# AdriaJ/pyxu

Hardware: AMD Instinct MI355X
Metric: solver iterations/s (PGD, TV-regularised deblur) (higher is better)
Workload: dtype f32; 1 GPU; PGD 2048x2048 Gaussian(sigma=2) deblur + lam*env_mu(L21 o Grad) TV, PositiveOrthant; images_per_gpu=1, stop_crit=MaxIter | RelError, fused_m_step=True, pgd_launch=x, x_prev, H^T y -> x_new (tile kernel), parallelism=independent images x1 (one per rank)

## Files before the change

include/pyxu_amd.h:

```cpp
#ifndef PYXU_AMD_H
#define PYXU_AMD_H

#include <stddef.h>
#include <stdint.h>

#ifdef __cplusplus
extern "C" {
#endif

#define PXA_F32 0
#define PXA_F64 1

#define PXA_OK 0
#define PXA_ERR_ARG (-1)
#define PXA_ERR_DTYPE (-2)
#define PXA_ERR_UNSUPPORTED (-3)

#define PXA_MAX_DIM 4
#define PXA_MAX_TAPS 64

#define PXA_MODE_CONSTANT 0
#define PXA_MODE_WRAP 1
#define PXA_MODE_REFLECT 2
#define PXA_MODE_SYMMETRIC 3
// ... 233 lines not shown
int pxa_pgd_tv2d_plan_step(void* plan, double a, double tau, double prox_w, const void* x, const void* x_prev,
                           const void* hty, void* x_new, double* partials, const void* x_ref, double* rel_values,
                           uint32_t* rel_flags, uint32_t seq, void* stream);
int pxa_pgd_tv2d_plan_step_fold(void* plan, double a, double tau, double prox_w, const void* x, const void* x_prev,
                                const void* hty, void* x_new, double* partials, const void* x_ref, double* rel_values,
                                uint32_t* rel_flags, uint32_t seq, void* stream);
int pxa_pgd_tv2d_plan_step_wfold(void* plan, double a, double tau, double prox_w, const void* x, const void* x_prev,
                                 const void* hty, void* x_new, double* partials, double* rel_values, uint32_t* rel_flags,
                                 uint32_t seq, void* stream);
int pxa_pgd_tv2d_plan_step_wpub(void* plan, double a, double tau, double prox_w, const void* x, const void* x_prev,
                                const void* hty, void* x_new, double* partials, const double* prev_partials,
                                double* rel_values, uint32_t* rel_flags, uint32_t seq, void* stream);
int pxa_pgd_tv2d_plan_free(void* plan);
int pxa_pgd_tv2d_last_kernel(void);
int pxa_pgd_tile_trace(uint64_t* host_out, int n);
int pxa_pgd_tv2d_step(int dtype, int64_t stack, int64_t y_images, int64_t n0, int64_t n1, int nt0, const int32_t* off0,
                      const double* coef0, int nt1, const int32_t* off1, const double* coef1, double h0, double h1,
                      double lam, double mu, double a, double tau, int prox, double prox_w, const void* x,
                      const void* x_prev, const void* hty, void* x_new, double* partials, const void* x_ref,
                      void* stream);


int pxa_fft(int dtype, int ndim, const int64_t* shape, int naxes, const int* axes, int64_t stack, int inverse,
            const void* in, void* out, void* stream);
size_t pxa_fft_workspace_bytes(int dtype, int ndim, const int64_t* shape, int naxes, const int* axes, int64_t stack);
int pxa_fft_ex(int dtype, int ndim, const int64_t* shape, int naxes, const int* axes, int64_t stack, int inverse,
               const void* in, void* out, void* work, void* stream);
int pxa_complex_mul(int dtype, int64_t n, int64_t nb, const void* a, const void* b, int conj_b, void* out,
                    void* stream);
int pxa_real_to_complex(int dtype, int64_t n, const void* x, void* z, void* stream);
// ... 35 lines not shown

int pxa_pds_slab_primal(int dtype, int algo, const int64_t* geom, const int32_t* ntaps, const int32_t* offs,
                        const double* coefs, const double* diff, const double* scal, int prox, int h_kind,
                        const void* x, const void* u, const void* z, const void* hty, void* x_out, void* u_out,
                        void* work_q, void* work_w, const int64_t* ghost, const void* src_lo, const void* src_hi,
                        const void* z_lo, const void* z_hi, int nseg, void* stream);
int pxa_pds_slab_dual(int dtype, int relax, const int64_t* geom, const double* diff, double sigma, double lam,
                      double rho, int h_kind, const void* w, const void* w_hi, int64_t w_hi_depth, const void* z,
                      void* z_out, void* stream);

int pxa_pds_step_la(int dtype, int algo, const int64_t* geom, const int32_t* ntaps, const int32_t* offs,
                    const double* coefs, const double* diff, const double* scal, int prox, int h_kind, int primed,
                    void* x, const void* u, const void* z, const void* hty, void* x_out, void* u_out, void* z_out,
                    void* work_q, void* work_kt, void* work_w, int nseg, void* stream);

#ifdef __cplusplus
}
#endif

#endif
```

pyxu_amd/_lib.py:

```python
import ctypes as ct
import os
import threading

__all__ = ["lib", "check", "BackendUnavailable", "LIB_PATH", "EXPORTS"]

LIB_PATH = os.environ.get("PXA_LIB_PATH") or os.path.join(os.path.dirname(os.path.abspath(__file__)), "libpyxu_amd.so")

i32, i64, f64, vp, sz = ct.c_int, ct.c_int64, ct.c_double, ct.c_void_p, ct.c_size_t
P_i64 = ct.POINTER(ct.c_int64)
P_i32 = ct.POINTER(ct.c_int32)
P_int = ct.POINTER(ct.c_int)
P_f64 = ct.POINTER(ct.c_double)

EXPORTS = {
    "pxa_version": (ct.c_char_p, []),
    "pxa_error_string": (ct.c_char_p, [i32]),
    "pxa_abi_version": (i32, []),
    "pxa_tuning": (i32, [i32, i32]),
    "pxa_axpby": (i32, [i32, i64, f64, vp, f64, vp, vp, vp]),
    "pxa_axpby_bcast": (i32, [i32, i64, f64, vp, f64, vp, i64, vp, vp]),
    "pxa_axpy_rows": (i32, [i32, i64, i64, vp, f64, vp, vp, vp, vp]),
    "pxa_row_ratio": (i32, [i32, i64, vp, vp, vp, vp]),
    "pxa_lincomb3": (i32, [i32, i64, f64, vp, f64, vp, f64, vp, vp, vp]),
    "pxa_extrapolate": (i32, [i32, i64, f64, vp, vp, vp, vp]),
# ... 56 lines not shown
    "pxa_dense_normal_pdot": (i32, [i32, i64, i64, vp, vp, f64, f64, vp, vp, vp, vp]),
    "pxa_dense_normal_pdot_pfold": (i32, [i32, i64, i64, vp, vp, vp, vp, vp, vp, vp, vp, vp, ct.c_uint32, f64, f64, vp, vp,
                                          vp, vp]),
    "pxa_copy2d": (i32, [i32, i64, i64, vp, i64, i64, vp, i64, i32, vp]),
    "pxa_unary": (i32, [i32, i32, i64, vp, vp, vp]),
    "pxa_binary": (i32, [i32, i32, i64, vp, f64, vp, f64, vp, vp]),
    "pxa_where": (i32, [i32, i64, vp, vp, f64, vp, f64, vp, vp]),
    "pxa_cast": (i32, [i32, i32, i64, vp, vp, vp]),
    "pxa_isnan": (i32, [i32, i64, vp, vp, vp]),
    "pxa_bool_reduce": (i32, [i64, i32, vp, vp, vp]),
    "pxa_set_diag": (i32, [i32, i64, i64, i64, f64, vp, vp]),
    "pxa_transpose": (i32, [i32, i64, i64, vp, vp, vp]),
    "pxa_dir_contract": (i32, [i32, i64, i64, i64, i64, i64, vp, i64, vp, vp, i32, vp]),
    "pxa_pgd_tv2d_partials_count": (i32, [i64, i64, i64]),
    "pxa_pgd_tv2d_last_kernel": (i32, []),
    "pxa_pgd_tile_trace": (i32, [vp, i32]),
    "pxa_pgd_tv2d_plan": (i32, [i32, i64, i64, i64, i64, i32, P_i32, P_f64, i32, P_i32, P_f64, f64, f64, f64, f64, i32,
                                ct.POINTER(vp)]),
    "pxa_pgd_tv2d_plan_step": (i32, [vp, f64, f64, f64, vp, vp, vp, vp, vp, vp, vp, vp, ct.c_uint32, vp]),
    "pxa_pgd_tv2d_plan_step_fold": (i32, [vp, f64, f64, f64, vp, vp, vp, vp, vp, vp, vp, vp, ct.c_uint32, vp]),
    "pxa_pgd_tv2d_plan_step_wfold": (i32, [vp, f64, f64, f64, vp, vp, vp, vp, vp, vp, vp, ct.c_uint32, vp]),
    "pxa_pgd_tv2d_plan_step_wpub": (i32, [vp, f64, f64, f64, vp, vp, vp, vp, vp, vp, vp, vp, ct.c_uint32, vp]),
    "pxa_pgd_tv2d_plan_free": (i32, [vp]),
    "pxa_pgd_tv2d_step": (
        i32,
        [i32, i64, i64, i64, i64, i32, P_i32, P_f64, i32, P_i32, P_f64, f64, f64, f64, f64, f64, f64, i32, f64,
         vp, vp, vp, vp, vp, vp, vp],
    ),
    "pxa_fft": (i32, [i32, i32, P_i64, i32, P_int, i64, i32, vp, vp, vp]),
    "pxa_fft_workspace_bytes": (sz, [i32, i32, P_i64, i32, P_int, i64]),
    "pxa_fft_ex": (i32, [i32, i32, P_i64, i32, P_int, i64, i32, vp, vp, vp, vp]),
# ... 106 lines not shown
```

pyxu_amd/csrc/pgd_tv2d.hip:

```cpp
#include "tile2d.hpp"
#include <type_traits>

#ifndef PXA_PGD_PRIO
#define PXA_PGD_PRIO 1
#endif
#ifndef PXA_PGD_PRIO_EPI
#define PXA_PGD_PRIO_EPI 0
#endif
#ifndef PXA_PGD_PRIO_FIN
#define PXA_PGD_PRIO_FIN 0
#endif

#ifndef PXA_PROBES
#define PXA_PROBES 0
#endif

namespace pxa {
namespace {

using namespace tile2d;
constexpr bool kProbes = PXA_PROBES != 0;


template <typename T>
// ... 12 lines not shown
  int diag;
  const T* xref;
  double* fold_vals;
  unsigned* fold_flags;
  unsigned* counter;
  unsigned fold_seq;
  int64_t fold_rows, fold_per_row;
  int win_part;
  const double* pub_src;
  double* pub_vals;
  unsigned* pub_flags;
  unsigned pub_seq;
};


constexpr int kTraceWords = 4 * 4 * 8;
__device__ unsigned long long g_tile_trace[kTraceWords];

template <typename T>
__device__ inline T tv_weight(T n2, T lam, T mu, T inv_mu) {
  const T n = sqrt(n2);
  return lam / (n > mu ? n : mu);
}
template <>
__device__ inline float tv_weight<float>(float n2, float lam, float mu, float inv_mu) {
  const float r = __builtin_amdgcn_rsqf(n2);
  return lam * __builtin_fminf(r, inv_mu);
}

template <typename T, int R>
struct Window {
  using L = Layout<T, R>;
// ... 59 lines not shown
    for (int i = 0; i < L::N0; ++i)
      if (cnt[i] != 1) return false;
    return true;
  }
  static_assert(covers_once(), "the window order is a bijection onto the AR x NGA window vectors");

  T xv[K0][L::V], pv[K0][L::V];
};

__device__ inline void wave_lane(int lt, int& wv, int& ln) {
  wv = __builtin_amdgcn_readfirstlane(lt >> 6);
  __builtin_assume(wv >= 0 && wv < kThreads / 64);
  ln = lt & 63;
}

constexpr int kMaxInteriorN1 = 1 << 22;
template <typename T>
__device__ inline T* lane_ptr(T* img, int row0, int col0, int n1, int ru, unsigned voff) {
  T* base = img + ((int64_t)row0 * n1 + col0) + ru * n1;
  using C = std::conditional_t<std::is_const_v<T>, const char, char>;
  return reinterpret_cast<T*>(reinterpret_cast<C*>(base) + (size_t)voff);
}

template <typename T, int R, bool EDGE>
__device__ inline void win_issue(const PgdParams<T>& p, int ty0, int tx0, const T* __restrict__ xs,
                                 const T* __restrict__ xps, Window<T, R>& w, int lt) {
  using L = Layout<T, R>;
  using W = Window<T, R>;
  constexpr int V = L::V;
  constexpr int CA = L::CA;
  const int n0 = p.n0, n1 = p.n1;
  int wv, ln;
  wave_lane(lt, wv, ln);
#pragma unroll
  for (int k = 0; k < W::K0; ++k) {
    int rl, gl, ru, gu;
    if (W::item(k, wv, ln, rl, gl, ru, gu)) {
      if (!EDGE) {
        const unsigned voff = (unsigned)(rl * n1 + V * gl) * (unsigned)sizeof(T);
        ld_vec<T, V>(lane_ptr<const T>(xs, ty0 - 2 * R, tx0 - CA + V * gu, n1, ru, voff), w.xv[k]);
        if (kProbes && (p.diag & 256)) {
#pragma unroll
          for (int v = 0; v < V; ++v) w.pv[k][v] = w.xv[k][v];
        } else {
          ld_vec<T, V>(lane_ptr<const T>(xps, ty0 - 2 * R, tx0 - CA + V * gu, n1, ru, voff), w.pv[k]);
        }
        continue;
      }
      const int gr = ty0 - 2 * R + rl + ru, gc = tx0 - CA + V * (gl + gu);
      if (gr >= 0 && gr < n0 && p.vec_ok && gc >= 0 && gc + V <= n1) {
        ld_vec<T, V>(xs + (int64_t)gr * n1 + gc, w.xv[k]);
        ld_vec<T, V>(xps + (int64_t)gr * n1 + gc, w.pv[k]);
      } else {
// ... 21 lines not shown
    if (W::item(k, wv, ln, rl, gl, ru, gu)) {
      T out[V];
#pragma unroll
      for (int v = 0; v < V; ++v) out[v] = fma(w.xv[k][v] - w.pv[k][v], p.a, w.xv[k][v]);
      st_vec<T, V>(A + (rl * L::AP + V * gl) + (ru * L::AP + V * gu), out);
    }
  }
}

template <typename T, int R>
__host__ __device__ constexpr int pt_pitch() {
  if constexpr (sizeof(T) == 4) return BlockB<T, R>::PTP;
  else return Layout<T, R>::PTP;
}

template <typename T, int R, bool EDGE, int D = 0>
__device__ inline void pass_a(const PgdParams<T>& p, const T* A, T* PT, const T* KT, int ty0, int tid = threadIdx.x) {
  using L = Layout<T, R>;
  constexpr int V = L::V;
  constexpr int KA = cdiv(L::NPA, kThreads);
  const bool edge_rows = EDGE && (ty0 < R || ty0 + TY > p.n0 - R);
#pragma unroll
  for (int k = 0; k < KA; ++k) {
    const int it = tid + k * kThreads;
    if (it < L::NPA) {
      const int a = it % L::NA, b = it / L::NA;
      T acc[V][V];
      sweep<T, R, V, L::AP, D>(A + (V * a) * L::AP + V * b, p.g0, acc);
      if (edge_rows) ghost_fix<T, R, V, L::AP>(ty0 + V * a, p.n0, ty0 - 2 * R, A + V * b, p.k0, KT, acc);
#pragma unroll
      for (int v = 0; v < V; ++v) {
        T colv[V];
#pragma unroll
        for (int u = 0; u < V; ++u) colv[u] = acc[u][v];
        st_vec<T, V>(PT + (V * b + v) * pt_pitch<T, R>() + V * a, colv);
      }
    }
  }
}

__device__ inline void st_pair(float* p, float a, float b) { *reinterpret_cast<float2*>(p) = make_float2(a, b); }

constexpr int kTvxP0 = 40;
template <typename T, int R>
constexpr int kTvxFloats = 9 * kTvxP0 + 9 * BlockB<T, R>::WR;

template <typename T, int R, bool EDGE>
__device__ inline void tv_block(const PgdParams<T>& p, T* A, int ty0, int tx0, int wv, int ln, T (&yc)[2][4],
                                T (&tv)[2][4]) {
  using L = Layout<T, R>;
  using B = BlockB<T, R>;
  constexpr int CA = L::CA, AP = L::AP;
  constexpr bool kExchange = (2 * R - 1) * AP >= 2 * kTvxFloats<T, R>;
  const int n0 = p.n0, n1 = p.n1;
  int rpl, cil, wr0, wc0;
  B::item(wv, ln, rpl, cil, wr0, wc0);
  const int r0 = wr0 + 2 * rpl, c0 = wc0 + 4 * cil;
  const T* own = A + (r0 + 2 * R) * AP + CA + c0;
  auto qat = [&](T yc_, T ydn, T yrt, int gr, int gc, T& q0, T& q1) {
    const T v0 = fma(p.g0a, yc_, p.g0b * ydn);
    const T v1 = fma(p.g1a, yc_, p.g1b * yrt);
    T w = tv_weight<T>(fma(v0, v0, v1 * v1), p.lam, p.mu, p.inv_mu);
    if (EDGE && !(gr >= 0 && gr < n0 && gc >= 0 && gc < n1)) w = T(0);
    q0 = v0 * w;
    q1 = v1 * w;
  };
  if constexpr (kExchange) {
    T y[3][5];
#pragma unroll
    for (int r = 0; r < 3; ++r) {
      T m[4];
      ld_vec<T, 4>(own + r * AP, m);
#pragma unroll
      for (int w = 0; w < 4; ++w) y[r][w] = m[w];
    }
#pragma unroll
    for (int r = 0; r < 2; ++r) {
      T hi[2];
// ... 6 lines not shown
      for (int w = 0; w < 4; ++w) yc[u][w] = y[u][w];
    if (!p.tv) return;
    T q0[2][4], q1[2][4];
#pragma unroll
    for (int u = 0; u < 2; ++u)
#pragma unroll
      for (int w = 0; w < 4; ++w)
        qat(y[u][w], y[u + 1][w], y[u][w + 1], ty0 + r0 + u, tx0 + c0 + w, q0[u][w], q1[u][w]);
    T* E0 = (wv < 2 ? A : A + (TY + 2 * R + 1) * AP) + (wv & 1) * kTvxFloats<T, R>;
    T* E1 = E0 + 9 * kTvxP0;
    if (ln < 48) {
      T hq0, hq1;
      if (ln < 32) {
        const int tc = wc0 + ln;
        const T* h = A + (wr0 - 1 + 2 * R) * AP + CA + tc;
        qat(h[0], h[AP], h[1], ty0 + wr0 - 1, tx0 + tc, hq0, hq1);
        E0[ln] = hq0;
      } else {
        const int j = ln - 32, tc = wc0 - 1;
        const T* h = A + (wr0 + j + 2 * R) * AP + CA + tc;
        qat(h[0], h[AP], h[1], ty0 + wr0 + j, tx0 + tc, hq0, hq1);
        E1[j] = hq1;
      }
    }
    st_vec<T, 4>(E0 + (rpl + 1) * kTvxP0 + 4 * cil, q0[1]);
    st_pair(E1 + (cil + 1) * B::WR + 2 * rpl, q1[0][3], q1[1][3]);
    __builtin_amdgcn_wave_barrier();
    asm volatile("" ::: "memory");
    T up[4], left[2];
    ld_vec<T, 4>(E0 + rpl * kTvxP0 + 4 * cil, up);
    ld_pair<T>(E1 + cil * B::WR + 2 * rpl, left);
#pragma unroll
    for (int u = 0; u < 2; ++u)
#pragma unroll
      for (int w = 0; w < 4; ++w) {
        const T qa = u == 0 ? up[w] : q0[0][w];
// ... 2 lines not shown
        const T t1 = fma(p.g1b, ql, p.g1a * q1[u][w]);
        tv[u][w] = t0 + t1;
      }
  } else {
    auto yrow = [&](int r, T(&y)[6]) {
      const T* arow = own + (r - 1) * AP;
      T m[4];
      ld_vec<T, 4>(arow, m);
      y[0] = arow[-1];
#pragma unroll
      for (int w = 0; w < 4; ++w) y[w + 1] = m[w];
      y[5] = arow[4];
    };
    auto qrow = [&](int r, const T(&yr)[6], const T(&yn)[6], T(&q0)[5], T(&q1)[5]) {
#pragma unroll
      for (int c = 0; c < 5; ++c) qat(yr[c], yn[c], yr[c + 1], ty0 + r0 - 1 + r, tx0 + c0 - 1 + c, q0[c], q1[c]);
    };
    T yr[6], yn[6];
    yrow(0, yr);
    yrow(1, yn);
    T qp0[5], qp1[5];
    if (p.tv) qrow(0, yr, yn, qp0, qp1);
#pragma unroll
    for (int u = 0; u < 2; ++u) {
#pragma unroll
      for (int c = 0; c < 6; ++c) yr[c] = yn[c];
      yrow(u + 2, yn);
#pragma unroll
      for (int w = 0; w < 4; ++w) yc[u][w] = yr[w + 1];
      if (p.tv) {
        T qc0[5], qc1[5];
// ... 188 lines not shown
#pragma unroll
  for (int off = 32; off > 0; off >>= 1) {
    part_d += __shfl_down(part_d, off, 64);
    part_x += __shfl_down(part_x, off, 64);
  }
  if ((threadIdx.x & 63) == 0) {
    __hip_atomic_store(partials + 2 * slot, part_d, __ATOMIC_RELAXED, __HIP_MEMORY_SCOPE_AGENT);
    __hip_atomic_store(partials + 2 * slot + 1, part_x, __ATOMIC_RELAXED, __HIP_MEMORY_SCOPE_AGENT);
  }
}

template <int R>
constexpr bool kRowsLiveB = R >= 4;
constexpr int kRingB = 4;

template <typename T, int R, bool EDGE, typename Mark>
__device__ inline void pass_b_blocks(const PgdParams<T>& p, T* A, const T* PT, const T* KT, const T* GH, int ty0, int tx0,
                                     const T* __restrict__ bs, const T* __restrict__ xrs, T* __restrict__ xns,
                                     bool want_part, double& part_d, double& part_x, int tid, Mark&& tmark) {
  using L = Layout<T, R>;
  using B = BlockB<T, R>;
  constexpr int CA = L::CA, PTP = B::PTP;
  const int n0 = p.n0, n1 = p.n1;
  const bool edge_cols = EDGE && (tx0 < R || tx0 + TX > n1 - R);
  int wv, ln;
  wave_lane(tid, wv, ln);
  int rpl, cil, wr0, wc0;
  B::item(wv, ln, rpl, cil, wr0, wc0);
  const int r0 = wr0 + 2 * rpl, c0 = wc0 + 4 * cil;
  auto voff = [&](int q) { return (unsigned)((2 * rpl + q) * n1 + 4 * cil) * (unsigned)sizeof(T); };
  auto load_rows = [&](const T* __restrict__ src, T(&v)[2][4]) {
#pragma unroll
    for (int q = 0; q < 2; ++q) {
      const int gr = ty0 + r0 + q, gc = tx0 + c0;
      if (!EDGE) {
        ld_vec<T, 4>(lane_ptr<const T>(src, ty0, tx0 + wc0, n1, wr0, voff(q)), v[q]);
      } else if (vec_inside(p, gr, gc)) {
// ... 14 lines not shown
    } else {
      load_rows(bs, bv);
    }
  };
  T yc[2][4], tv[2][4], acc[4][2];
  if (kProbes && (p.diag & 64)) {
#pragma unroll
    for (int q = 0; q < 2; ++q)
#pragma unroll
      for (int w = 0; w < 4; ++w) yc[q][w] = tv[q][w] = acc[w][q] = A[tid + q * 64 + w];
    load_epilogue();
    tmark(5);
  } else {
    const T* src = PT + (CA - 2 * R + c0) * PTP + r0;
    if constexpr (kRowsLiveB<R>) {
      tv_block<T, R, EDGE>(p, A, ty0, tx0, wv, ln, yc, tv);
      tmark(5);
      load_epilogue();
      sweep_w<T, R, 4, 2, PTP>(src, p.g1, acc);
    } else {
      T g1[4 * R + 1];
#pragma unroll
      for (int k = 0; k <= 4 * R; ++k) {
        g1[k] = p.g1[k];
        asm volatile("" : "+s"(g1[k]));
      }
      RowSweep<T, R, 4, 2, PTP, kRingB> sw;
      tv_block<T, R, EDGE>(p, A, ty0, tx0, wv, ln, yc, tv);
      tmark(5);
      load_epilogue();
      sw.start(src);
      sw.run(src, g1, acc);
    }
    if (edge_cols) ghost_fix_pre_w<T, R, 4, 2, TY>(tx0 + c0, n1, r0, GH, KT + kKT, acc);
  }
  if (want_part) load_rows(xrs, xv);
  tmark(6);
#pragma unroll
  for (int q = 0; q < 2; ++q) {
    T g[4];
#pragma unroll
    for (int w = 0; w < 4; ++w) g[w] = p.tv ? acc[w][q] + tv[q][w] : acc[w][q];
    if (kProbes && (p.diag & 1024)) {
      if (g[0] + yc[q][0] + bv[q][0] == T(-12345)) xns[0] = T(0);
      continue;
    }
    T* vdst = EDGE ? nullptr : lane_ptr<T>(xns, ty0, tx0 + wc0, n1, wr0, voff(q));
    finish_vec<T, EDGE>(p, ty0 + r0 + q, tx0 + c0, g, bv[q], yc[q], xv[q], xns, vdst, want_part, part_d, part_x);
  }
// ... 80 lines not shown
      ld_vec<T, V>(A + (r + 2 * R) * L::AP + L::CA + V * cq, y);
      if (kProbes && (p.diag & 1024)) {
        if (g[0] + y[0] + hb.v[s][0] == T(-12345)) xns[0] = T(0);
        continue;
      }
      T* vdst = EDGE ? nullptr : lane_ptr<T>(xns, ty0, tx0, n1, 0, stage_voff<T, R>(r0, cq, n1, s));
      finish_vec<T, EDGE>(p, ty0 + r, tx0 + V * cq, g, hb.v[s], y, hb.x[s], xns, vdst, want_part, part_d, part_x);
    }
  }
}

#ifndef PXA_PGD_SWEEP_DEPTH
#define PXA_PGD_SWEEP_DEPTH 0
#endif

template <typename T, int R, bool EDGE, int D>
__device__ inline void pgd_tile_body(const PgdParams<T>& p, unsigned char* smem, unsigned tile, int ty0, int tx0,
                                     const T* __restrict__ bs, T* __restrict__ xns, double* __restrict__ partials,
                                     const T* __restrict__ xrs, const int tid) {
  using L = Layout<T, R>;
  T* A = reinterpret_cast<T*>(smem);
  T* PT = A + L::AR * L::AP;
  T* KT = PT + L::AC * L::PTP;
  T* GH = reinterpret_cast<T*>(smem + kGhOff<T, R>);
  const int n1 = p.n1;
  const bool edge_cols = EDGE && (tx0 < R || tx0 + TX > n1 - R);
  double part_d = 0.0, part_x = 0.0;
  const bool want_part = partials != nullptr;
  const bool tracing = kProbes && (p.diag & 32) != 0;
  unsigned long long* ts = reinterpret_cast<unsigned long long*>(smem + kGhOff<T, R> + kGhBytes<T, R>);
  auto tmark = [&](int pt) {
    if (tracing && (tid & 63) == 0) ts[(tid >> 6) * 8 + pt] = clock64();
  };
  tmark(2);
  const bool skip_passes = kProbes && (p.diag & 64) != 0;
  if (!skip_passes) pass_a<T, R, EDGE, D>(p, A, PT, KT, ty0, tid);
  tmark(3);
  __syncthreads();
  if (edge_cols) {
    ghost_cols_coop<T, R, pt_pitch<T, R>()>(p.k1, PT, GH, tx0, n1, tid);
    __syncthreads();
  }
  tmark(4);
  if constexpr (sizeof(T) == 4) {
    pass_b_blocks<T, R, EDGE>(p, A, PT, KT, GH, ty0, tx0, bs, xrs, xns, want_part, part_d, part_x, tid, tmark);
  } else {
    pass_b_staged<T, R, EDGE, D>(p, A, PT, KT, GH, ty0, tx0, bs, xrs, xns, want_part, part_d, part_x, tid, tmark);
  }
  tmark(7);
  if (want_part) wave_partials(part_d, part_x, partials, tile * kPartWaves + (tid >> 6));
  const unsigned nb = gridDim.x, bid = blockIdx.x;
  if (tracing && (bid == 0 || bid == 9 || bid == nb / 2 + 8 || bid == nb - 1)) {
    __syncthreads();
    const int slot = bid == 0 ? 0 : bid == 9 ? 1 : bid == nb / 2 + 8 ? 2 : 3;
    if (tid < 32) g_tile_trace[slot * 32 + tid] = ts[tid];
  }
}


template <typename T, int R>
__device__ inline void win_partials(const Window<T, R>& w, double* __restrict__ partials, unsigned tile, const int tid) {
  using L = Layout<T, R>;
  double part_d = 0.0, part_x = 0.0;
#pragma unroll
  for (int k = 0; k < Window<T, R>::KI; ++k) {
#pragma unroll
    for (int v = 0; v < L::V; ++v) {
      const double dd = (double)w.xv[k][v] - (double)w.pv[k][v];
      part_d = fma(dd, dd, part_d);
      part_x = fma((double)w.pv[k][v], (double)w.pv[k][v], part_x);
    }
  }
  part_d = wave_sum_f64(part_d);
  part_x = wave_sum_f64(part_x);
  if ((tid & 63) == 0) {
    const unsigned slot = tile * kPartWaves + (tid >> 6);
    __hip_atomic_store(partials + 2 * slot, part_d, __ATOMIC_RELAXED, __HIP_MEMORY_SCOPE_AGENT);
    __hip_atomic_store(partials + 2 * slot + 1, part_x, __ATOMIC_RELAXED, __HIP_MEMORY_SCOPE_AGENT);
  }
}

template <typename T, int R, bool EDGE>
__device__ inline void pgd_tile(const PgdParams<T>& p, unsigned char* smem, unsigned tile, int ty0, int tx0,
                                const T* __restrict__ xs, const T* __restrict__ xps, const T* __restrict__ bs,
                                T* __restrict__ xns, double* __restrict__ partials, const T* __restrict__ xrs) {
  using L = Layout<T, R>;
  T* A = reinterpret_cast<T*>(smem);
  T* KT = A + L::AR * L::AP + L::AC * L::PTP;
  const int tid = threadIdx.x;
  if (EDGE && tid < 2 * R + 1) {
    KT[tid] = p.k0[tid];
    KT[kKT + tid] = p.k1[tid];
  }
  const bool tracing = kProbes && (p.diag & 32) != 0;
  unsigned long long* ts = reinterpret_cast<unsigned long long*>(smem + kGhOff<T, R> + kGhBytes<T, R>);
  auto tmark = [&](int pt) {
    if (tracing && (tid & 63) == 0) ts[(tid >> 6) * 8 + pt] = clock64();
  };
  tmark(0);
#if PXA_PGD_PRIO
  __builtin_amdgcn_s_setprio(PXA_PGD_PRIO);
#endif
  if (kProbes && (p.diag & 128)) {
    for (int i = tid; i < L::AR * L::AP; i += kThreads) A[i] = T(0);
  } else {
    Window<T, R> w;
    win_issue<T, R, EDGE>(p, ty0, tx0, xs, xps, w, tid);
    win_store<T, R>(p, A, w, tid);
    if (p.win_part && partials != nullptr) win_partials<T, R>(w, partials, tile, tid);
  }
#if PXA_PGD_PRIO
  __builtin_amdgcn_s_setprio(0);
#endif
  tmark(1);
  __syncthreads();
  int btid = tid;
  if constexpr (sizeof(T) == 8) asm volatile("" : "+v"(btid));
  pgd_tile_body<T, R, EDGE, PXA_PGD_SWEEP_DEPTH>(p, smem, tile, ty0, tx0, bs, xns, p.win_part ? nullptr : partials, xrs,
                                                 btid);
}

template <typename T>
__device__ inline void tail_fold(const PgdParams<T>& p, const double* __restrict__ partials) {
  __shared__ double red[kThreads / 64];
  __shared__ unsigned last;
  asm volatile("s_waitcnt vmcnt(0)" ::: "memory");
  __syncthreads();
  if (threadIdx.x == 0)
    last = __hip_atomic_fetch_add(p.counter, 1u, __ATOMIC_RELAXED, __HIP_MEMORY_SCOPE_AGENT) == gridDim.x - 1 ? 1u : 0u;
  __syncthreads();
  if (!last) return;
  auto ld = [](const double* a) { return __hip_atomic_load(a, __ATOMIC_RELAXED, __HIP_MEMORY_SCOPE_AGENT); };
  for (int64_t q = 0; q < 2 * p.fold_rows; ++q) {
// ... 23 lines not shown
  }
}

template <typename T, int R>
__global__ void __launch_bounds__(kThreads, 4) pgd_tv2d_kernel(PgdParams<T> p, const T* __restrict__ x,
                                                            const T* __restrict__ xp, const T* __restrict__ b,
                                                            T* __restrict__ xn, double* __restrict__ partials) {
  using L = Layout<T, R>;
  const unsigned pub = p.pub_src != nullptr ? 1u : 0u;
  if (pub && blockIdx.x == 0) {
    __shared__ double red[kThreads / 64];
    publish_prev<T>(p, red);
    return;
  }
  const unsigned vb = blockIdx.x - pub;
  extern __shared__ __align__(16) unsigned char smem_raw[];
  unsigned tile = xcd_tile(vb, p.ntiles);
  {
    const unsigned nb = p.ntiles, q8 = nb >> 3, r8 = nb & 7u, g8 = vb & 7u;
    if (g8 == 7u) {
      const unsigned lo = 7u * q8 + (r8 < 7u ? r8 : 7u), len = q8 + (7u < r8 ? 1u : 0u);
      tile = lo + (len - 1u - (tile - lo));
    }
  }
  const unsigned tpi = (unsigned)p.tiles0 * (unsigned)p.tiles1;
  const unsigned s = tile / tpi;
  const unsigned tr = tile - s * tpi;
  const unsigned trow = tr / (unsigned)p.tiles1;
  const int ty0 = (int)trow * TY, tx0 = (int)(tr - trow * (unsigned)p.tiles1) * TX;
  const int64_t img = (int64_t)p.n0 * p.n1;
  const T* xs = x + (int64_t)s * img;
  const T* xps = xp + (int64_t)s * img;
  const T* bs = b + (int64_t)(s % (unsigned)p.y_images) * img;
  T* xns = xn + (int64_t)s * img;
  const T* xrs = (p.xref != nullptr ? p.xref : x) + (int64_t)s * img;
  const bool interior = p.vec_ok && img <= 0x7fffffff && p.n1 <= kMaxInteriorN1 && ty0 - 2 * R >= 0 && ty0 + TY + 2 * R <= p.n0 &&
                        tx0 - L::CA >= 0 && tx0 + TX + L::CA <= p.n1;
  if (interior)
    pgd_tile<T, R, false>(p, smem_raw, tile, ty0, tx0, xs, xps, bs, xns, partials, xrs);
  else
    pgd_tile<T, R, true>(p, smem_raw, tile, ty0, tx0, xs, xps, bs, xns, partials, xrs);
  if (p.fold_vals != nullptr) tail_fold<T>(p, partials);
}

thread_local int g_last_pgd_kernel = 0;

template <typename T, int R>
int launch_pgd(const PgdParams<T>& p, const void* x, const void* xp, const void* b, void* xn, double* partials,
               hipStream_t s) {
  g_last_pgd_kernel = 1;
  const size_t smem = kGhOff<T, R> + kGhBytes<T, R> + ((p.diag & 32) ? 256 : 0);
  auto kern = pgd_tv2d_kernel<T, R>;
  static bool attr_set = false;
  if (!attr_set) {
    (void)hipFuncSetAttribute((const void*)kern, hipFuncAttributeMaxDynamicSharedMemorySize,
                              (int)(kGhOff<T, R> + kGhBytes<T, R> + 256));
    attr_set = true;
  }
  hipLaunchKernelGGL(kern, dim3(p.ntiles + (p.pub_src != nullptr ? 1u : 0u)), dim3(kThreads), smem, s, p, (const T*)x,
                     (const T*)xp, (const T*)b, (T*)xn, partials);
  return last_launch_status();
}


template <typename T>
int pgd_params(int64_t stack, int64_t y_images, int64_t n0, int64_t n1, int nt0, const int32_t* off0,
               const double* coef0, int nt1, const int32_t* off1, const double* coef1, double h0, double h1, double lam,
               double mu, int prox, PgdParams<T>& p, int& R) {
  PXA_CHECK_ARG(stack >= 1 && n0 >= 1 && n1 >= 1 && y_images >= 1 && stack % y_images == 0);
  PXA_CHECK_ARG(n0 <= 0x7fffffff && n1 <= 0x7fffffff);
  PXA_CHECK_ARG(prox >= 0 && prox <= 2);
// ... 94 lines not shown

using namespace pxa;

extern "C" {

int pxa_pgd_tv2d_last_kernel(void) { return g_last_pgd_kernel; }

int pxa_pgd_tile_trace(uint64_t* host_out, int n) {
  if (!kProbes) return PXA_ERR_UNSUPPORTED;
  if (!host_out || n < 0 || n > kTraceWords) return PXA_ERR_ARG;
  if (hipMemcpyFromSymbol(host_out, HIP_SYMBOL(g_tile_trace), (size_t)n * 8, 0, hipMemcpyDeviceToHost) != hipSuccess)
    return PXA_ERR_UNSUPPORTED;
  return PXA_OK;
}

int pxa_pgd_tv2d_partials_count(int64_t stack, int64_t n0, int64_t n1) {
  int64_t t = stack * ((n0 + TY - 1) / TY) * ((n1 + TX - 1) / TX) * kPartWaves;
  return (int)t;
}

int pxa_pgd_tv2d_plan(int dtype, int64_t stack, int64_t y_images, int64_t n0, int64_t n1, int nt0, const int32_t* off0,
                      const double* coef0, int nt1, const int32_t* off1, const double* coef1, double h0, double h1,
                      double lam, double mu, int prox, void** plan) {
  PXA_CHECK_ARG(plan != nullptr);
  *plan = nullptr;
  PgdPlan* pl = new PgdPlan();
  pl->dtype = dtype;
  int e = PXA_ERR_DTYPE;
  auto prepare = [&](auto& p) {
    e = pgd_params(stack, y_images, n0, n1, nt0, off0, coef0, nt1, off1, coef1, h0, h1, lam, mu, prox, p, pl->R);
    pl->fold_rows = p.fold_rows;
    pl->fold_per_row = p.fold_per_row;
  };
// ... 80 lines not shown
```

pyxu_amd/csrc/tile2d.hpp:

```cpp
#pragma once
#include "common.hpp"

namespace pxa {
namespace tile2d {

constexpr int TY = 32;
constexpr int TX = 64;
constexpr int kThreads = 256;
constexpr int kMaxR = 8;
constexpr int kMaxG = 4 * kMaxR + 1;
constexpr int kKT = 2 * kMaxR + 2;

__host__ __device__ constexpr int cdiv(int a, int b) { return (a + b - 1) / b; }
__host__ __device__ constexpr int rup(int a, int b) { return cdiv(a, b) * b; }

template <typename T, int R>
struct Layout {
  static constexpr int V = kVecN<T>;
  static constexpr bool F32 = sizeof(T) == 4;
  static constexpr int CA = rup(2 * R, V);
  static constexpr int AR = TY + 4 * R;
  static constexpr int AC = TX + 2 * CA;
  static constexpr int NGA = AC / V;
  static constexpr int NA = TY / V;
// ... 357 lines not shown
      const int i = i0 + o;
      if (i >= n || (side == 0 ? i >= R : i < n - R)) continue;
#pragma unroll
      for (int m = 0; m < R; ++m) {
        const int t = i - (pg + m);
        if (t < -R || t > R) continue;
        const T kk = kt[t + R];
        const auto* src = GH + (side * R + m) * GP + cc;
#pragma unroll
        for (int v = 0; v < W; ++v) acc[o][v] = fma(-kk, src[v], acc[o][v]);
      }
    }
  }
}

__device__ inline unsigned xcd_tile(unsigned bid, unsigned nb) {
  const unsigned q8 = nb >> 3, r8 = nb & 7u, g8 = bid & 7u;
  return g8 * q8 + (g8 < r8 ? g8 : r8) + (bid >> 3);
}

using TapWindow = double[2 * kMaxR + 1];
inline int tap_window(int nt, const int32_t* off, const double* coef, TapWindow& k) {
  for (double& v : k) v = 0.0;
  int R = 0;
  for (int q = 0; q < nt; ++q) R = abs(off[q]) > R ? abs(off[q]) : R;
  if (R > kMaxR) return -1;
  for (int q = 0; q < nt; ++q) k[off[q] + kMaxR] += coef[q];
  return R;
}

// ... 22 lines not shown
```

Before: 46540 image-iterations/s.

## Add specialised row/column border tile classes to avoid generic edge path in f32 PGD kernel

Splits f32 PGD tiles into four classes (interior, left/right column border, top/bottom row border, generic) and compiles specialised kernels for single-side border tiles. These use compile-time ghost subtraction from precomputed ghost rows/columns instead of the fully bounds-checked generic path. The aim is cheaper border tiles, at the cost of more template instantiations, code size and LDS for the ghost buffer (guarded by a static_assert on occupancy). It also adds probe-only timeline tracing and a host tile-class counting helper.

```diff
diff --git a/include/pyxu_amd.h b/include/pyxu_amd.h
--- a/include/pyxu_amd.h
+++ b/include/pyxu_amd.h
@@ -271,6 +271,7 @@
 int pxa_pgd_tv2d_plan_free(void* plan);
 int pxa_pgd_tv2d_last_kernel(void);
 int pxa_pgd_tile_trace(uint64_t* host_out, int n);
+int pxa_pgd_tile_timeline(uint64_t* host_out, int nwg);
 int pxa_pgd_tv2d_step(int dtype, int64_t stack, int64_t y_images, int64_t n0, int64_t n1, int nt0, const int32_t* off0,
                       const double* coef0, int nt1, const int32_t* off1, const double* coef1, double h0, double h1,
                       double lam, double mu, double a, double tau, int prox, double prox_w, const void* x,
@@ -336,6 +337,8 @@
                     void* x, const void* u, const void* z, const void* hty, void* x_out, void* u_out, void* z_out,
                     void* work_q, void* work_kt, void* work_w, int nseg, void* stream);
 
+int pxa_pgd_tv2d_tile_classes(int64_t stack, int64_t n0, int64_t n1, int R, int aligned, int64_t* counts);
+
 #ifdef __cplusplus
 }
 #endif
diff --git a/pyxu_amd/_lib.py b/pyxu_amd/_lib.py
--- a/pyxu_amd/_lib.py
+++ b/pyxu_amd/_lib.py
@@ -94,7 +94,9 @@
     "pxa_dir_contract": (i32, [i32, i64, i64, i64, i64, i64, vp, i64, vp, vp, i32, vp]),
     "pxa_pgd_tv2d_partials_count": (i32, [i64, i64, i64]),
     "pxa_pgd_tv2d_last_kernel": (i32, []),
+    "pxa_pgd_tv2d_tile_classes": (i32, [i64, i64, i64, i32, i32, P_i64]),
     "pxa_pgd_tile_trace": (i32, [vp, i32]),
+    "pxa_pgd_tile_timeline": (i32, [vp, i32]),
     "pxa_pgd_tv2d_plan": (i32, [i32, i64, i64, i64, i64, i32, P_i32, P_f64, i32, P_i32, P_f64, f64, f64, f64, f64, i32,
                                 ct.POINTER(vp)]),
     "pxa_pgd_tv2d_plan_step": (i32, [vp, f64, f64, f64, vp, vp, vp, vp, vp, vp, vp, vp, ct.c_uint32, vp]),
diff --git a/pyxu_amd/csrc/pgd_tv2d.hip b/pyxu_amd/csrc/pgd_tv2d.hip
--- a/pyxu_amd/csrc/pgd_tv2d.hip
+++ b/pyxu_amd/csrc/pgd_tv2d.hip
@@ -50,8 +50,12 @@
 };
 
 
-constexpr int kTraceWords = 4 * 4 * 8;
+constexpr int kTraceWords = 5 * 4 * 8;
 __device__ unsigned long long g_tile_trace[kTraceWords];
+#if PXA_PROBES
+constexpr unsigned kTimelineWgs = 1u << 14;
+__device__ unsigned long long g_tile_timeline[3 * kTimelineWgs];
+#endif
 
 template <typename T>
 __device__ inline T tv_weight(T n2, T lam, T mu, T inv_mu) {
@@ -141,7 +145,6 @@
   ln = lt & 63;
 }
 
-constexpr int kMaxInteriorN1 = 1 << 22;
 template <typename T>
 __device__ inline T* lane_ptr(T* img, int row0, int col0, int n1, int ru, unsigned voff) {
   T* base = img + ((int64_t)row0 * n1 + col0) + ru * n1;
@@ -149,21 +152,38 @@
   return reinterpret_cast<T*>(reinterpret_cast<C*>(base) + (size_t)voff);
 }
 
-template <typename T, int R, bool EDGE>
+template <int C>
+__device__ inline int tile_side(int ty0, int tx0) {
+  return __builtin_amdgcn_readfirstlane(C == kTileCol ? (tx0 == 0 ? 0 : 1) : (ty0 == 0 ? 0 : 1));
+}
+
+template <typename T, int R, int C>
 __device__ inline void win_issue(const PgdParams<T>& p, int ty0, int tx0, const T* __restrict__ xs,
                                  const T* __restrict__ xps, Window<T, R>& w, int lt) {
   using L = Layout<T, R>;
   using W = Window<T, R>;
   constexpr int V = L::V;
   constexpr int CA = L::CA;
+  constexpr bool EDGE = C == kTileGeneric;
   const int n0 = p.n0, n1 = p.n1;
   int wv, ln;
   wave_lane(lt, wv, ln);
+  const int side = tile_side<C>(ty0, tx0);
 #pragma unroll
   for (int k = 0; k < W::K0; ++k) {
     int rl, gl, ru, gu;
     if (W::item(k, wv, ln, rl, gl, ru, gu)) {
       if (!EDGE) {
+        if ((C == kTileCol || C == kTileRow) && k >= W::KI) {
+          const int r = rl + ru, g = gl + gu;
+          const bool outside = C == kTileCol ? (side == 0 ? g < W::CV : g >= W::CV + W::TV)
+                                             : (side == 0 ? r < 2 * R : r >= 2 * R + TY);
+          if (outside) {
+#pragma unroll
+            for (int v = 0; v < V; ++v) w.xv[k][v] = w.pv[k][v] = T(0);
+            continue;
+          }
+        }
         const unsigned voff = (unsigned)(rl * n1 + V * gl) * (unsigned)sizeof(T);
         ld_vec<T, V>(lane_ptr<const T>(xs, ty0 - 2 * R, tx0 - CA + V * gu, n1, ru, voff), w.xv[k]);
         if (kProbes && (p.diag & 256)) {
@@ -215,11 +235,38 @@
   else return Layout<T, R>::PTP;
 }
 
-template <typename T, int R, bool EDGE, int D = 0>
-__device__ inline void pass_a(const PgdParams<T>& p, const T* A, T* PT, const T* KT, int ty0, int tid = threadIdx.x) {
+template <typename T, int R>
+constexpr size_t kPgdGhBytes =
+    sizeof(T) == 4 && (size_t)R * Layout<T, R>::AC * sizeof(T) > kGhBytes<T, R> ? (size_t)R * Layout<T, R>::AC * sizeof(T)
+                                                                                  : kGhBytes<T, R>;
+
+template <typename T, int R>
+__device__ inline void ghost_rows_coop(const PgdParams<T>& p, const T* A, T* GH, int side, int a, int b) {
+  using L = Layout<T, R>;
+  constexpr int V = L::V;
+  static_assert(R <= L::NA, "one ghost row per lane of a column group");
+  if (a < R) {
+    const T* src = A + ((side == 0 ? 0 : TY + R) + a) * L::AP + V * b;
+    T gh[V];
+#pragma unroll
+    for (int v = 0; v < V; ++v) gh[v] = T(0);
+#pragma unroll
+    for (int s = 0; s <= 2 * R; ++s) {
+      T w[V];
+      ld_vec<T, V>(src + s * L::AP, w);
+#pragma unroll
+      for (int v = 0; v < V; ++v) gh[v] = fma(p.k0[s], w[v], gh[v]);
+    }
+    st_vec<T, V>(GH + (b * R + a) * V, gh);
+  }
+}
+
+template <typename T, int R, int C, int D = 0>
+__device__ inline void pass_a(const PgdParams<T>& p, const T* A, T* PT, const T* KT, T* GH, int ty0, int tid = threadIdx.x) {
   using L = Layout<T, R>;
   constexpr int V = L::V;
   constexpr int KA = cdiv(L::NPA, kThreads);
+  constexpr bool EDGE = C == kTileGeneric;
   const bool edge_rows = EDGE && (ty0 < R || ty0 + TY > p.n0 - R);
 #pragma unroll
   for (int k = 0; k < KA; ++k) {
@@ -227,7 +274,25 @@
     if (it < L::NPA) {
       const int a = it % L::NA, b = it / L::NA;
       T acc[V][V];
-      sweep<T, R, V, L::AP, D>(A + (V * a) * L::AP + V * b, p.g0, acc);
+      if constexpr (C == kTileRow) {
+        static_assert(KA == 1 && L::NPA % L::NA == 0 && 64 % L::NA == 0, "a column group is NA lanes of one wave");
+        static_assert(V == 4 && L::NA == 8 && R <= 8, "the row groups within R of a border: two on each side");
+        const int side = tile_side<C>(ty0, 0);
+        ghost_rows_coop<T, R>(p, A, GH, side, a, b);
+        sweep<T, R, V, L::AP, D>(A + (V * a) * L::AP + V * b, p.g0, acc);
+        __builtin_amdgcn_wave_barrier();
+        asm volatile("" ::: "memory");
+        const T* gh = GH + b * R * V;
+        if (side == 0) {
+          if (a == 0) ghost_sub<T, R, V, V, V, false, 0>(p.k0, gh, acc);
+          if (R > V && a == 1) ghost_sub<T, R, V, V, V, false, V>(p.k0, gh, acc);
+        } else {
+          if (a == L::NA - 1) ghost_sub<T, R, V, V, V, true, V - 1>(p.k0, gh, acc);
+          if (R > V && a == L::NA - 2) ghost_sub<T, R, V, V, V, true, 2 * V - 1>(p.k0, gh, acc);
+        }
+      } else {
+        sweep<T, R, V, L::AP, D>(A + (V * a) * L::AP + V * b, p.g0, acc);
+      }
       if (edge_rows) ghost_fix<T, R, V, L::AP>(ty0 + V * a, p.n0, ty0 - 2 * R, A + V * b, p.k0, KT, acc);
 #pragma unroll
       for (int v = 0; v < V; ++v) {
@@ -246,23 +311,26 @@
 template <typename T, int R>
 constexpr int kTvxFloats = 9 * kTvxP0 + 9 * BlockB<T, R>::WR;
 
-template <typename T, int R, bool EDGE>
+template <typename T, int R, int C>
 __device__ inline void tv_block(const PgdParams<T>& p, T* A, int ty0, int tx0, int wv, int ln, T (&yc)[2][4],
                                 T (&tv)[2][4]) {
   using L = Layout<T, R>;
   using B = BlockB<T, R>;
   constexpr int CA = L::CA, AP = L::AP;
+  constexpr bool EDGE = C == kTileGeneric;
+  const bool first = (C == kTileCol || C == kTileRow) && tile_side<C>(ty0, tx0) == 0;
   constexpr bool kExchange = (2 * R - 1) * AP >= 2 * kTvxFloats<T, R>;
   const int n0 = p.n0, n1 = p.n1;
   int rpl, cil, wr0, wc0;
   B::item(wv, ln, rpl, cil, wr0, wc0);
   const int r0 = wr0 + 2 * rpl, c0 = wc0 + 4 * cil;
   const T* own = A + (r0 + 2 * R) * AP + CA + c0;
-  auto qat = [&](T yc_, T ydn, T yrt, int gr, int gc, T& q0, T& q1) {
+  auto qat = [&](T yc_, T ydn, T yrt, int gr, int gc, T& q0, T& q1, bool zq = false) {
     const T v0 = fma(p.g0a, yc_, p.g0b * ydn);
     const T v1 = fma(p.g1a, yc_, p.g1b * yrt);
     T w = tv_weight<T>(fma(v0, v0, v1 * v1), p.lam, p.mu, p.inv_mu);
     if (EDGE && !(gr >= 0 && gr < n0 && gc >= 0 && gc < n1)) w = T(0);
+    if (zq) w = T(0);
     q0 = v0 * w;
     q1 = v1 * w;
   };
@@ -299,12 +367,12 @@
       if (ln < 32) {
         const int tc = wc0 + ln;
         const T* h = A + (wr0 - 1 + 2 * R) * AP + CA + tc;
-        qat(h[0], h[AP], h[1], ty0 + wr0 - 1, tx0 + tc, hq0, hq1);
+        qat(h[0], h[AP], h[1], ty0 + wr0 - 1, tx0 + tc, hq0, hq1, C == kTileRow && first && wr0 == 0);
         E0[ln] = hq0;
       } else {
         const int j = ln - 32, tc = wc0 - 1;
         const T* h = A + (wr0 + j + 2 * R) * AP + CA + tc;
-        qat(h[0], h[AP], h[1], ty0 + wr0 + j, tx0 + tc, hq0, hq1);
+        qat(h[0], h[AP], h[1], ty0 + wr0 + j, tx0 + tc, hq0, hq1, C == kTileCol && first && wc0 == 0);
         E1[j] = hq1;
       }
     }
@@ -337,7 +405,9 @@
     };
     auto qrow = [&](int r, const T(&yr)[6], const T(&yn)[6], T(&q0)[5], T(&q1)[5]) {
 #pragma unroll
-      for (int c = 0; c < 5; ++c) qat(yr[c], yn[c], yr[c + 1], ty0 + r0 - 1 + r, tx0 + c0 - 1 + c, q0[c], q1[c]);
+      for (int c = 0; c < 5; ++c)
+        qat(yr[c], yn[c], yr[c + 1], ty0 + r0 - 1 + r, tx0 + c0 - 1 + c, q0[c], q1[c],
+            first && (C == kTileCol ? c == 0 && c0 == 0 : r == 0 && r0 == 0));
     };
     T yr[6], yn[6];
     yrow(0, yr);
@@ -556,13 +626,14 @@
 constexpr bool kRowsLiveB = R >= 4;
 constexpr int kRingB = 4;
 
-template <typename T, int R, bool EDGE, typename Mark>
+template <typename T, int R, int C, typename Mark>
 __device__ inline void pass_b_blocks(const PgdParams<T>& p, T* A, const T* PT, const T* KT, const T* GH, int ty0, int tx0,
                                      const T* __restrict__ bs, const T* __restrict__ xrs, T* __restrict__ xns,
                                      bool want_part, double& part_d, double& part_x, int tid, Mark&& tmark) {
   using L = Layout<T, R>;
   using B = BlockB<T, R>;
   constexpr int CA = L::CA, PTP = B::PTP;
+  constexpr bool EDGE = C == kTileGeneric;
   const int n0 = p.n0, n1 = p.n1;
   const bool edge_cols = EDGE && (tx0 < R || tx0 + TX > n1 - R);
   int wv, ln;
@@ -607,7 +678,7 @@
   } else {
     const T* src = PT + (CA - 2 * R + c0) * PTP + r0;
     if constexpr (kRowsLiveB<R>) {
-      tv_block<T, R, EDGE>(p, A, ty0, tx0, wv, ln, yc, tv);
+      tv_block<T, R, C>(p, A, ty0, tx0, wv, ln, yc, tv);
       tmark(5);
       load_epilogue();
       sweep_w<T, R, 4, 2, PTP>(src, p.g1, acc);
@@ -619,13 +690,23 @@
         asm volatile("" : "+s"(g1[k]));
       }
       RowSweep<T, R, 4, 2, PTP, kRingB> sw;
-      tv_block<T, R, EDGE>(p, A, ty0, tx0, wv, ln, yc, tv);
+      tv_block<T, R, C>(p, A, ty0, tx0, wv, ln, yc, tv);
       tmark(5);
       load_epilogue();
       sw.start(src);
       sw.run(src, g1, acc);
     }
     if (edge_cols) ghost_fix_pre_w<T, R, 4, 2, TY>(tx0 + c0, n1, r0, GH, KT + kKT, acc);
+    if constexpr (C == kTileCol) {
+      static_assert(R <= 8, "columns within R of a border: two blocks on each side");
+      if (tile_side<C>(ty0, tx0) == 0) {
+        if (c0 == 0) ghost_sub<T, R, 4, 2, TY, false, 0>(p.k1, GH + r0, acc);
+        if (R > 4 && c0 == 4) ghost_sub<T, R, 4, 2, TY, false, 4>(p.k1, GH + r0, acc);
+      } else {
+        if (c0 == TX - 4) ghost_sub<T, R, 4, 2, TY, true, 3>(p.k1, GH + R * TY + r0, acc);
+        if (R > 4 && c0 == TX - 8) ghost_sub<T, R, 4, 2, TY, true, 7>(p.k1, GH + R * TY + r0, acc);
+      }
+    }
   }
   if (want_part) load_rows(xrs, xv);
   tmark(6);
@@ -736,7 +817,7 @@
 #define PXA_PGD_SWEEP_DEPTH 0
 #endif
 
-template <typename T, int R, bool EDGE, int D>
+template <typename T, int R, int C, int D>
 __device__ inline void pgd_tile_body(const PgdParams<T>& p, unsigned char* smem, unsigned tile, int ty0, int tx0,
                                      const T* __restrict__ bs, T* __restrict__ xns, double* __restrict__ partials,
                                      const T* __restrict__ xrs, const int tid) {
@@ -745,36 +826,41 @@
   T* PT = A + L::AR * L::AP;
   T* KT = PT + L::AC * L::PTP;
   T* GH = reinterpret_cast<T*>(smem + kGhOff<T, R>);
+  constexpr bool EDGE = C == kTileGeneric;
   const int n1 = p.n1;
   const bool edge_cols = EDGE && (tx0 < R || tx0 + TX > n1 - R);
   double part_d = 0.0, part_x = 0.0;
   const bool want_part = partials != nullptr;
   const bool tracing = kProbes && (p.diag & 32) != 0;
-  unsigned long long* ts = reinterpret_cast<unsigned long long*>(smem + kGhOff<T, R> + kGhBytes<T, R>);
+  unsigned long long* ts = reinterpret_cast<unsigned long long*>(smem + kGhOff<T, R> + kPgdGhBytes<T, R>);
   auto tmark = [&](int pt) {
     if (tracing && (tid & 63) == 0) ts[(tid >> 6) * 8 + pt] = clock64();
   };
   tmark(2);
   const bool skip_passes = kProbes && (p.diag & 64) != 0;
-  if (!skip_passes) pass_a<T, R, EDGE, D>(p, A, PT, KT, ty0, tid);
+  if (!skip_passes) pass_a<T, R, C, D>(p, A, PT, KT, GH, ty0, tid);
   tmark(3);
   __syncthreads();
   if (edge_cols) {
     ghost_cols_coop<T, R, pt_pitch<T, R>()>(p.k1, PT, GH, tx0, n1, tid);
     __syncthreads();
   }
+  if constexpr (C == kTileCol) {
+    ghost_cols_side<T, R, pt_pitch<T, R>()>(p.k1, PT, GH, tile_side<C>(ty0, tx0), tid);
+    __syncthreads();
+  }
   tmark(4);
   if constexpr (sizeof(T) == 4) {
-    pass_b_blocks<T, R, EDGE>(p, A, PT, KT, GH, ty0, tx0, bs, xrs, xns, want_part, part_d, part_x, tid, tmark);
+    pass_b_blocks<T, R, C>(p, A, PT, KT, GH, ty0, tx0, bs, xrs, xns, want_part, part_d, part_x, tid, tmark);
   } else {
     pass_b_staged<T, R, EDGE, D>(p, A, PT, KT, GH, ty0, tx0, bs, xrs, xns, want_part, part_d, part_x, tid, tmark);
   }
   tmark(7);
   if (want_part) wave_partials(part_d, part_x, partials, tile * kPartWaves + (tid >> 6));
   const unsigned nb = gridDim.x, bid = blockIdx.x;
-  if (tracing && (bid == 0 || bid == 9 || bid == nb / 2 + 8 || bid == nb - 1)) {
+  if (tracing && (bid == 0 || bid == 9 || bid == nb / 2 + 8 || bid == nb - 1 || bid == 8)) {
     __syncthreads();
-    const int slot = bid == 0 ? 0 : bid == 9 ? 1 : bid == nb / 2 + 8 ? 2 : 3;
+    const int slot = bid == 0 ? 0 : bid == 9 ? 1 : bid == nb / 2 + 8 ? 2 : bid == nb - 1 ? 3 : 4;
     if (tid < 32) g_tile_trace[slot * 32 + tid] = ts[tid];
   }
 }
@@ -802,7 +888,7 @@
   }
 }
 
-template <typename T, int R, bool EDGE>
+template <typename T, int R, int C>
 __device__ inline void pgd_tile(const PgdParams<T>& p, unsigned char* smem, unsigned tile, int ty0, int tx0,
                                 const T* __restrict__ xs, const T* __restrict__ xps, const T* __restrict__ bs,
                                 T* __restrict__ xns, double* __restrict__ partials, const T* __restrict__ xrs) {
@@ -810,12 +896,13 @@
   T* A = reinterpret_cast<T*>(smem);
   T* KT = A + L::AR * L::AP + L::AC * L::PTP;
   const int tid = threadIdx.x;
+  constexpr bool EDGE = C == kTileGeneric;
   if (EDGE && tid < 2 * R + 1) {
     KT[tid] = p.k0[tid];
     KT[kKT + tid] = p.k1[tid];
   }
   const bool tracing = kProbes && (p.diag & 32) != 0;
-  unsigned long long* ts = reinterpret_cast<unsigned long long*>(smem + kGhOff<T, R> + kGhBytes<T, R>);
+  unsigned long long* ts = reinterpret_cast<unsigned long long*>(smem + kGhOff<T, R> + kPgdGhBytes<T, R>);
   auto tmark = [&](int pt) {
     if (tracing && (tid & 63) == 0) ts[(tid >> 6) * 8 + pt] = clock64();
   };
@@ -827,7 +914,7 @@
     for (int i = tid; i < L::AR * L::AP; i += kThreads) A[i] = T(0);
   } else {
     Window<T, R> w;
-    win_issue<T, R, EDGE>(p, ty0, tx0, xs, xps, w, tid);
+    win_issue<T, R, C>(p, ty0, tx0, xs, xps, w, tid);
     win_store<T, R>(p, A, w, tid);
     if (p.win_part && partials != nullptr) win_partials<T, R>(w, partials, tile, tid);
   }
@@ -838,7 +925,7 @@
   __syncthreads();
   int btid = tid;
   if constexpr (sizeof(T) == 8) asm volatile("" : "+v"(btid));
-  pgd_tile_body<T, R, EDGE, PXA_PGD_SWEEP_DEPTH>(p, smem, tile, ty0, tx0, bs, xns, p.win_part ? nullptr : partials, xrs,
+  pgd_tile_body<T, R, C, PXA_PGD_SWEEP_DEPTH>(p, smem, tile, ty0, tx0, bs, xns, p.win_part ? nullptr : partials, xrs,
                                                  btid);
 }
 
@@ -892,6 +979,8 @@
     return;
   }
   const unsigned vb = blockIdx.x - pub;
+  const bool timeline = kProbes && (p.diag & 32) != 0;
+  [[maybe_unused]] const unsigned long long tl0 = timeline ? clock64() : 0ull;
   extern __shared__ __align__(16) unsigned char smem_raw[];
   unsigned tile = xcd_tile(vb, p.ntiles);
   {
@@ -912,12 +1001,40 @@
   const T* bs = b + (int64_t)(s % (unsigned)p.y_images) * img;
   T* xns = xn + (int64_t)s * img;
   const T* xrs = (p.xref != nullptr ? p.xref : x) + (int64_t)s * img;
-  const bool interior = p.vec_ok && img <= 0x7fffffff && p.n1 <= kMaxInteriorN1 && ty0 - 2 * R >= 0 && ty0 + TY + 2 * R <= p.n0 &&
-                        tx0 - L::CA >= 0 && tx0 + TX + L::CA <= p.n1;
-  if (interior)
-    pgd_tile<T, R, false>(p, smem_raw, tile, ty0, tx0, xs, xps, bs, xns, partials, xrs);
-  else
-    pgd_tile<T, R, true>(p, smem_raw, tile, ty0, tx0, xs, xps, bs, xns, partials, xrs);
+  [[maybe_unused]] int tl_cls = kTileGeneric;
+  if constexpr (sizeof(T) == 4) {
+    int cls = __builtin_amdgcn_readfirstlane(tile_class(p.n0, p.n1, ty0, tx0, R, L::CA, p.vec_ok));
+    if (kProbes && (p.diag & 2048) && cls != kTileInterior) cls = kTileGeneric;
+    if (kProbes) tl_cls = cls;
+    if (cls == kTileInterior)
+      pgd_tile<T, R, kTileInterior>(p, smem_raw, tile, ty0, tx0, xs, xps, bs, xns, partials, xrs);
+    else if (cls == kTileCol)
+      pgd_tile<T, R, kTileCol>(p, smem_raw, tile, ty0, tx0, xs, xps, bs, xns, partials, xrs);
+    else if (cls == kTileRow)
+      pgd_tile<T, R, kTileRow>(p, smem_raw, tile, ty0, tx0, xs, xps, bs, xns, partials, xrs);
+    else
+      pgd_tile<T, R, kTileGeneric>(p, smem_raw, tile, ty0, tx0, xs, xps, bs, xns, partials, xrs);
+  } else {
+    const bool interior = p.vec_ok && img <= 0x7fffffff && p.n1 <= kMaxInteriorN1 && ty0 - 2 * R >= 0 && ty0 + TY + 2 * R <= p.n0 &&
+                          tx0 - L::CA >= 0 && tx0 + TX + L::CA <= p.n1;
+    if (kProbes && interior) tl_cls = kTileInterior;
+    if (interior)
+      pgd_tile<T, R, kTileInterior>(p, smem_raw, tile, ty0, tx0, xs, xps, bs, xns, partials, xrs);
+    else
+      pgd_tile<T, R, kTileGeneric>(p, smem_raw, tile, ty0, tx0, xs, xps, bs, xns, partials, xrs);
+  }
+#if PXA_PROBES
+  if (timeline) {
+    __syncthreads();
+    if (threadIdx.x == 0 && vb < kTimelineWgs) {
+      g_tile_timeline[3 * vb] = tl0;
+      g_tile_timeline[3 * vb + 1] = clock64();
+      const unsigned xcc = __builtin_amdgcn_s_getreg((3 << 11) | 20), hw = __builtin_amdgcn_s_getreg((15 << 11) | 4);
+      g_tile_timeline[3 * vb + 2] = (unsigned long long)tile | (unsigned long long)tl_cls << 32 |
+                                    (unsigned long long)(xcc & 15u) << 36 | (unsigned long long)(hw & 0xffffu) << 40;
+    }
+  }
+#endif
   if (p.fold_vals != nullptr) tail_fold<T>(p, partials);
 }
 
@@ -927,12 +1044,14 @@
 int launch_pgd(const PgdParams<T>& p, const void* x, const void* xp, const void* b, void* xn, double* partials,
                hipStream_t s) {
   g_last_pgd_kernel = 1;
-  const size_t smem = kGhOff<T, R> + kGhBytes<T, R> + ((p.diag & 32) ? 256 : 0);
+  constexpr size_t kLds = 160 * 1024;
+  static_assert(kLds / (kGhOff<T, R> + kPgdGhBytes<T, R>) == kLds / (kGhOff<T, R> + kGhBytes<T, R>), "LDS occupancy step lost");
+  const size_t smem = kGhOff<T, R> + kPgdGhBytes<T, R> + ((p.diag & 32) ? 256 : 0);
   auto kern = pgd_tv2d_kernel<T, R>;
   static bool attr_set = false;
   if (!attr_set) {
     (void)hipFuncSetAttribute((const void*)kern, hipFuncAttributeMaxDynamicSharedMemorySize,
-                              (int)(kGhOff<T, R> + kGhBytes<T, R> + 256));
+                              (int)(kGhOff<T, R> + kPgdGhBytes<T, R> + 256));
     attr_set = true;
   }
   hipLaunchKernelGGL(kern, dim3(p.ntiles + (p.pub_src != nullptr ? 1u : 0u)), dim3(kThreads), smem, s, p, (const T*)x,
@@ -1057,9 +1176,32 @@
   return PXA_OK;
 }
 
+int pxa_pgd_tile_timeline(uint64_t* host_out, int nwg) {
+#if PXA_PROBES
+  if (!host_out || nwg < 0 || (unsigned)nwg > kTimelineWgs) return PXA_ERR_ARG;
+  if (hipMemcpyFromSymbol(host_out, HIP_SYMBOL(g_tile_timeline), (size_t)nwg * 24, 0, hipMemcpyDeviceToHost) != hipSuccess)
+    return PXA_ERR_UNSUPPORTED;
+  return PXA_OK;
+#else
+  (void)host_out, (void)nwg;
+  return PXA_ERR_UNSUPPORTED;
+#endif
+}
+
 int pxa_pgd_tv2d_partials_count(int64_t stack, int64_t n0, int64_t n1) {
   int64_t t = stack * ((n0 + TY - 1) / TY) * ((n1 + TX - 1) / TX) * kPartWaves;
   return (int)t;
+}
+
+int pxa_pgd_tv2d_tile_classes(int64_t stack, int64_t n0, int64_t n1, int R, int aligned, int64_t* counts) {
+  PXA_CHECK_ARG(counts != nullptr && stack >= 1 && n0 >= 1 && n1 >= 1 && n0 <= 0x7fffffff && n1 <= 0x7fffffff);
+  PXA_CHECK_ARG(R >= 1 && R <= kMaxR);
+  constexpr int V = kVecN<float>;
+  const bool vec_ok = aligned != 0 && n1 % V == 0;
+  for (int c = 0; c < 4; ++c) counts[c] = 0;
+  for (int64_t ty0 = 0; ty0 < n0; ty0 += TY)
+    for (int64_t tx0 = 0; tx0 < n1; tx0 += TX) counts[tile_class((int)n0, (int)n1, (int)ty0, (int)tx0, R, rup(2 * R, V), vec_ok)] += stack;
+  return PXA_OK;
 }
 
 int pxa_pgd_tv2d_plan(int dtype, int64_t stack, int64_t y_images, int64_t n0, int64_t n1, int nt0, const int32_t* off0,
diff --git a/pyxu_amd/csrc/tile2d.hpp b/pyxu_amd/csrc/tile2d.hpp
--- a/pyxu_amd/csrc/tile2d.hpp
+++ b/pyxu_amd/csrc/tile2d.hpp
@@ -395,6 +395,52 @@
   }
 }
 
+enum TileClass : int { kTileInterior = 0, kTileCol = 1, kTileRow = 2, kTileGeneric = 3 };
+constexpr int kMaxInteriorN1 = 1 << 22;
+__host__ __device__ inline int tile_class(int n0, int n1, int ty0, int tx0, int R, int CA, bool vec_ok) {
+  if (!vec_ok || (int64_t)n0 * n1 > 0x7fffffff || n1 > kMaxInteriorN1) return kTileGeneric;
+  const bool up = ty0 - 2 * R >= 0, down = ty0 + TY + 2 * R <= n0;
+  const bool left = tx0 - CA >= 0, right = tx0 + TX + CA <= n1;
+  if (up && down && left && right) return kTileInterior;
+  if (up && down && ((tx0 == 0 && right) || (tx0 + TX == n1 && left))) return kTileCol;
+  if (left && right && ((ty0 == 0 && down) || (ty0 + TY == n0 && up))) return kTileRow;
+  return kTileGeneric;
+}
+
+template <typename T, int R, int PTP>
+__device__ inline void ghost_cols_side(const T* __restrict__ k, const T* PT, T* GH, int side, int lt) {
+  using L = Layout<T, R>;
+  static_assert(L::CA >= 2 * R, "ghost columns and their taps inside the window");
+  for (int t = lt; t < R * TY; t += kThreads) {
+    const int m = t / TY, r = t % TY;
+    const int row = (side == 0 ? L::CA - R : L::CA + TX) + m;
+    T g = T(0);
+#pragma unroll
+    for (int q = -R; q <= R; ++q) g = fma(k[q + R], PT[(row + q) * PTP + r], g);
+    GH[(side * R + m) * TY + r] = g;
+  }
+}
+
+template <typename T, int R, int NO, int W, int GP, bool FAR, int P0>
+__device__ inline void ghost_sub(const T* __restrict__ k, const T* __restrict__ gh, T (&acc)[NO][W]) {
+#pragma unroll
+  for (int o = 0; o < NO; ++o) {
+    const int d = FAR ? P0 - o : P0 + o;
+    if (d < 0 || d >= R) continue;
+#pragma unroll
+    for (int m = 0; m < R; ++m) {
+      const int t = FAR ? -(d + 1) - m : d + R - m;
+      if (t < -R || t > R) continue;
+      const T kk = k[t + R];
+      T g[W];
+#pragma unroll
+      for (int v = 0; v < W; ++v) g[v] = gh[m * GP + v];
+#pragma unroll
+      for (int v = 0; v < W; ++v) acc[o][v] = fma(-kk, g[v], acc[o][v]);
+    }
+  }
+}
+
 __device__ inline unsigned xcd_tile(unsigned bid, unsigned nb) {
   const unsigned q8 = nb >> 3, r8 = nb & 7u, g8 = bid & 7u;
   return g8 * q8 + (g8 < r8 ? g8 : r8) + (bid >> 3);
```

Result: faster. 55330 image-iterations/s, median of 6 (+18.9%).
